# yu-changqian/TorchSeg

Hardware: AMD Instinct MI355X
Metric: training images/sec (1024x1024) BiSeNet-R18 (higher is better)
Workload: dtype bf16

## Files before the change

### torchseg_amd/csrc/conv3wrw.hip

```cpp
#include "tsg_common.h"
#include <stdlib.h>

namespace tsg {

typedef __attribute__((ext_vector_type(8))) __bf16 bf16x8;
typedef __attribute__((ext_vector_type(16))) float f32x16;
typedef uint32_t __attribute__((may_alias)) lds_u32;
typedef uint16_t __attribute__((may_alias)) lds_u16;
typedef bf16x8 __attribute__((may_alias)) lds_bf16x8;

constexpr int W3_C = 64;
constexpr int W3_N = 9 * W3_C;
constexpr int W3_TH = 4, W3_TW = 32;
constexpr int W3_PR = W3_TH + 2;
constexpr int W3_PP = (W3_TW + 2) / 2;
constexpr int W3_RD = 20;
constexpr int W3_CS = 121;
constexpr int W3_COPY = W3_C * W3_CS;
constexpr int W3_DS = 68;
constexpr int W3_NCH = 8 * W3_PR * W3_PP;
constexpr int W3_NU = (W3_NCH + 255) / 256;
constexpr int W3_NPART = 256;

struct W3Geom { int B, H, W, tiles_h, tiles_w, ntiles, two; };

__global__ __launch_bounds__(256) void conv3_wrw_k(const bf16_t* __restrict__ x, const bf16_t* __restrict__ dy,
                                                   float* __restrict__ part, W3Geom g) {
  extern __shared__ __attribute__((aligned(16))) uint32_t lds[];
  lds_u32* dyT = reinterpret_cast<lds_u32*>(lds);
  lds_u32* xT = dyT + W3_C * W3_DS;
  lds_u16* xT16 = reinterpret_cast<lds_u16*>(xT);
  const int tid = threadIdx.x, lane = tid & 63, wave = tid >> 6, half = lane >> 5, n = lane & 31;
  const int wm = wave >> 1, wh = wave & 1;

  const int spp = tid & 15, strow = (tid >> 4) & 1, spart = tid >> 5;
  int xoff[W3_NU], xrc[W3_NU], xdst[W3_NU];
#pragma unroll
  for (int u = 0; u < W3_NU; ++u) {
    const int q = tid + 256 * u;
    const int cpart = q / (W3_PR * W3_PP), rem = q % (W3_PR * W3_PP), r = rem / W3_PP, pc = rem % W3_PP;
    xrc[u] = q < W3_NCH ? (r | ((2 * pc) << 8)) : -1;
    xoff[u] = ((r - 1) * g.W + 2 * pc - 1) * W3_C + cpart * 8;
    xdst[u] = (cpart * 8) * W3_CS + r * W3_RD + pc;
  }
  const lds_u32* afrag = dyT + (32 * wm + n) * W3_DS + 4 * half;
  const lds_u32* bfrag = xT + (32 * wh + n) * W3_CS + 4 * half;

  f32x16 acc[9];
#pragma unroll
  for (int t = 0; t < 9; ++t)
#pragma unroll
    for (int r = 0; r < 16; ++r) acc[t][r] = 0.f;

  uint4 rd[4];
  uint4 rx[W3_NU][2];
  auto fetch = [&](int tile) {
    const int ow0 = (tile % g.tiles_w) * W3_TW, oh0 = ((tile / g.tiles_w) % g.tiles_h) * W3_TH;
    const int b = tile / (g.tiles_w * g.tiles_h);
    const int64_t org = (((int64_t)b * g.H + oh0) * g.W + ow0) * W3_C;
    const bf16_t* dt = dy + org + ((int64_t)strow * g.W + 2 * spp) * W3_C + spart * 8;
#pragma unroll
    for (int rs = 0; rs < 2; ++rs)
#pragma unroll
      for (int px = 0; px < 2; ++px)
        rd[rs * 2 + px] = (oh0 + strow + 2 * rs < g.H && ow0 + 2 * spp + px < g.W)
                              ? *reinterpret_cast<const uint4*>(dt + ((int64_t)rs * 2 * g.W + px) * W3_C)
                              : make_uint4(0, 0, 0, 0);
    const bf16_t* xo = x + org;
#pragma unroll
    for (int u = 0; u < W3_NU; ++u) {
      const int ih = oh0 - 1 + (xrc[u] & 0xff), iw = ow0 - 1 + (xrc[u] >> 8);
      const bool rowok = xrc[u] >= 0 && ih >= 0 && ih < g.H;
      rx[u][0] = (rowok && iw >= 0 && iw < g.W) ? *reinterpret_cast<const uint4*>(xo + xoff[u]) : make_uint4(0, 0, 0, 0);
      rx[u][1] = (rowok && iw + 1 >= 0 && iw + 1 < g.W) ? *reinterpret_cast<const uint4*>(xo + xoff[u] + W3_C)
                                                         : make_uint4(0, 0, 0, 0);
    }
  };

  int tile = blockIdx.x;
  if (tile < g.ntiles) fetch(tile);
  for (; tile < g.ntiles; tile += gridDim.x) {
    __syncthreads();
#pragma unroll
    for (int rs = 0; rs < 2; ++rs) {
      const uint32_t wa[4] = {rd[2 * rs].x, rd[2 * rs].y, rd[2 * rs].z, rd[2 * rs].w};
      const uint32_t wb[4] = {rd[2 * rs + 1].x, rd[2 * rs + 1].y, rd[2 * rs + 1].z, rd[2 * rs + 1].w};
      lds_u32* drow = dyT + (spart * 8) * W3_DS + 16 * (strow + 2 * rs) + spp;
#pragma unroll
      for (int e = 0; e < 8; ++e)
        drow[e * W3_DS] = (e & 1) ? ((wa[e >> 1] >> 16) | (wb[e >> 1] & 0xffff0000u))
                                  : ((wa[e >> 1] & 0xffffu) | (wb[e >> 1] << 16));
    }
#pragma unroll
    for (int u = 0; u < W3_NU; ++u) {
      if (u < W3_NU - 1 || xrc[u] >= 0) {
        const uint32_t wa[4] = {rx[u][0].x, rx[u][0].y, rx[u][0].z, rx[u][0].w};
        const uint32_t wb[4] = {rx[u][1].x, rx[u][1].y, rx[u][1].z, rx[u][1].w};
#pragma unroll
        for (int e = 0; e < 8; ++e) {
          const uint32_t a = (e & 1) ? (wa[e >> 1] >> 16) : (wa[e >> 1] & 0xffffu);
          const uint32_t b2 = (e & 1) ? (wb[e >> 1] >> 16) : (wb[e >> 1] & 0xffffu);
          const int d = xdst[u] + e * W3_CS;
          xT[d] = a | (b2 << 16);
          xT16[2 * (W3_COPY + d) + 1] = (uint16_t)a;
          xT16[2 * (W3_COPY + d) + g.two] = (uint16_t)b2;
        }
      }
    }
    __syncthreads();
    if (tile + (int)gridDim.x < g.ntiles) fetch(tile + gridDim.x);
#pragma unroll
    for (int ks = 0; ks < 8; ++ks) {
      const bf16x8 fa = *reinterpret_cast<const lds_bf16x8*>(afrag + ks * 8);
#pragma unroll
      for (int kh = 0; kh < 3; ++kh)
#pragma unroll
        for (int kw = 0; kw < 3; ++kw) {
          const int sg = kw & 1;
          const lds_u32* q = bfrag + sg * W3_COPY + ((ks >> 1) + kh) * W3_RD + (ks & 1) * 8 + ((kw + sg) >> 1);
          union { uint32_t u[4]; bf16x8 v; } fb;
          fb.u[0] = q[0]; fb.u[1] = q[1]; fb.u[2] = q[2]; fb.u[3] = q[3];
          acc[kh * 3 + kw] = __builtin_amdgcn_mfma_f32_32x32x16_bf16(fa, fb.v, acc[kh * 3 + kw], 0, 0, 0);
        }
    }
  }
  float* out = part + (int64_t)blockIdx.x * W3_C * W3_N;
#pragma unroll
  for (int t = 0; t < 9; ++t)
#pragma unroll
    for (int r = 0; r < 16; ++r) {
      const int oc = 32 * wm + (r & 3) + 8 * (r >> 2) + 4 * half;
      out[oc * W3_N + t * W3_C + 32 * wh + n] = acc[t][r];
    }
}

typedef short v4i16 __attribute__((ext_vector_type(4)));
typedef v4i16 __attribute__((address_space(3))) lds_v4i16;

constexpr int T3_RBE = 96;
constexpr int T3_PC = W3_TW + 2;
constexpr int T3_NPX = W3_PR * T3_PC;
constexpr int T3_DY = W3_TH * W3_TW * T3_RBE;
constexpr int T3_XU = (T3_NPX * 8 + 255) / 256;
constexpr size_t T3_LDS = (size_t)(T3_DY + T3_NPX * T3_RBE) * sizeof(bf16_t);

__device__ __forceinline__ uint4 w3_affine_relu(uint4 v, const float* __restrict__ ab, int part8) {
  uint32_t w[4] = {v.x, v.y, v.z, v.w};
  const float4 a0 = *reinterpret_cast<const float4*>(ab + part8), a1 = *reinterpret_cast<const float4*>(ab + part8 + 4);
  const float4 b0 = *reinterpret_cast<const float4*>(ab + W3_C + part8), b1 = *reinterpret_cast<const float4*>(ab + W3_C + part8 + 4);
  const float a[8] = {a0.x, a0.y, a0.z, a0.w, a1.x, a1.y, a1.z, a1.w};
  const float b[8] = {b0.x, b0.y, b0.z, b0.w, b1.x, b1.y, b1.z, b1.w};
#pragma unroll
  for (int i = 0; i < 4; ++i) {
    const float x0 = __uint_as_float(w[i] << 16), x1 = __uint_as_float(w[i] & 0xffff0000u);
    const float y0 = fmaf(x0, a[2 * i], b[2 * i]), y1 = fmaf(x1, a[2 * i + 1], b[2 * i + 1]);
    w[i] = pack2_bf16(y0 > 0.f ? y0 : 0.f, y1 > 0.f ? y1 : 0.f);
  }
  return make_uint4(w[0], w[1], w[2], w[3]);
}

template <bool AFF>
__global__ __launch_bounds__(256) void conv3_wrw_tr_k(const bf16_t* __restrict__ x, const bf16_t* __restrict__ dy,
                                                      float* __restrict__ part, W3Geom g, const float* __restrict__ in_ab) {
  __shared__ __attribute__((aligned(16))) float abs_[AFF ? 2 * W3_C : 4];
  if (AFF && threadIdx.x < 2 * W3_C) abs_[threadIdx.x] = in_ab[threadIdx.x];
  extern __shared__ __attribute__((aligned(16))) uint32_t lds[];
  bf16_t* dyL = reinterpret_cast<bf16_t*>(lds);
  bf16_t* xL = dyL + T3_DY;
  const int tid = threadIdx.x, lane = tid & 63, wave = tid >> 6;
  const int wm = wave >> 1, wh = wave & 1;
  const int half = lane >> 5, sub = (lane >> 4) & 1, i16 = lane & 15;

  const int spart = tid & 7, spix = tid >> 3;
  int xr[T3_XU], xc[T3_XU];
#pragma unroll
  for (int u = 0; u < T3_XU; ++u) {
    const int pp = spix + 32 * u;
    xr[u] = pp < T3_NPX ? pp / T3_PC : -1;
    xc[u] = pp % T3_PC;
  }
  const int fbase = (8 * half + (i16 >> 2)) * T3_RBE + 16 * sub + 4 * (i16 & 3);
  const lds_v4i16* afr = (const lds_v4i16*)(dyL + fbase + 32 * wm);
  const lds_v4i16* bfr = (const lds_v4i16*)(xL + fbase + 32 * wh);

  f32x16 acc[9];
#pragma unroll
  for (int t = 0; t < 9; ++t)
#pragma unroll
    for (int r = 0; r < 16; ++r) acc[t][r] = 0.f;

  uint4 rd[W3_TH];
  uint4 rx[T3_XU];
  auto fetch = [&](int tile) {
    const int ow0 = (tile % g.tiles_w) * W3_TW, oh0 = ((tile / g.tiles_w) % g.tiles_h) * W3_TH;
    const int b = tile / (g.tiles_w * g.tiles_h);
    const int64_t org = (((int64_t)b * g.H + oh0) * g.W + ow0) * W3_C;
    const bf16_t* dt = dy + org + (int64_t)spix * W3_C + spart * 8;
#pragma unroll
    for (int u = 0; u < W3_TH; ++u)
      rd[u] = (oh0 + u < g.H && ow0 + spix < g.W) ? *reinterpret_cast<const uint4*>(dt + (int64_t)u * g.W * W3_C)
                                                  : make_uint4(0, 0, 0, 0);
    const bf16_t* xo = x + org + spart * 8;
#pragma unroll
    for (int u = 0; u < T3_XU; ++u) {
      const int ih = oh0 - 1 + xr[u], iw = ow0 - 1 + xc[u];
      rx[u] = (xr[u] >= 0 && ih >= 0 && ih < g.H && iw >= 0 && iw < g.W)
                  ? *reinterpret_cast<const uint4*>(xo + ((int64_t)(xr[u] - 1) * g.W + xc[u] - 1) * W3_C)
                  : make_uint4(0, 0, 0, 0);
    }
  };

  int tile = blockIdx.x;
  if (tile < g.ntiles) fetch(tile);
  for (; tile < g.ntiles; tile += gridDim.x) {
    __syncthreads();
#pragma unroll
    for (int u = 0; u < W3_TH; ++u)
      *reinterpret_cast<uint4*>(dyL + (spix + 32 * u) * T3_RBE + spart * 8) = rd[u];
    const int cur_ow0 = (tile % g.tiles_w) * W3_TW, cur_oh0 = ((tile / g.tiles_w) % g.tiles_h) * W3_TH;
#pragma unroll
    for (int u = 0; u < T3_XU; ++u)
      if (u < T3_XU - 1 || xr[u] >= 0) {
        uint4 v = rx[u];
        if (AFF) {
          const int ih = cur_oh0 - 1 + xr[u], iw = cur_ow0 - 1 + xc[u];
          if (ih >= 0 && ih < g.H && iw >= 0 && iw < g.W) v = w3_affine_relu(v, abs_, spart * 8);
        }
        *reinterpret_cast<uint4*>(xL + (spix + 32 * u) * T3_RBE + spart * 8) = v;
      }
    __syncthreads();
    if (tile + (int)gridDim.x < g.ntiles) fetch(tile + gridDim.x);
#pragma unroll
    for (int ks = 0; ks < 8; ++ks) {
      union { v4i16 q[2]; bf16x8 v; } fa;
      fa.q[0] = __builtin_amdgcn_ds_read_tr16_b64_v4i16((lds_v4i16*)(afr + (ks * 16 + 0) * (T3_RBE / 4)));
      fa.q[1] = __builtin_amdgcn_ds_read_tr16_b64_v4i16((lds_v4i16*)(afr + (ks * 16 + 4) * (T3_RBE / 4)));
#pragma unroll
      for (int kh = 0; kh < 3; ++kh)
#pragma unroll
        for (int kw = 0; kw < 3; ++kw) {
          const int px = ((ks >> 1) + kh) * T3_PC + (ks & 1) * 16 + kw;
          union { v4i16 q[2]; bf16x8 v; } fb;
          fb.q[0] = __builtin_amdgcn_ds_read_tr16_b64_v4i16((lds_v4i16*)(bfr + (px + 0) * (T3_RBE / 4)));
          fb.q[1] = __builtin_amdgcn_ds_read_tr16_b64_v4i16((lds_v4i16*)(bfr + (px + 4) * (T3_RBE / 4)));
          acc[kh * 3 + kw] = __builtin_amdgcn_mfma_f32_32x32x16_bf16(fa.v, fb.v, acc[kh * 3 + kw], 0, 0, 0);
        }
    }
  }
  float* out = part + (int64_t)blockIdx.x * W3_C * W3_N;
#pragma unroll
  for (int t = 0; t < 9; ++t)
#pragma unroll
    for (int r = 0; r < 16; ++r) {
      const int oc = 32 * wm + (r & 3) + 8 * (r >> 2) + 4 * half;
      out[oc * W3_N + t * W3_C + 32 * wh + (lane & 31)] = acc[t][r];
    }
}

struct W3GenGeom {
  int B, H, W, tiles_h, tiles_w, ntiles;
  int Hin, Win;
  int Cin, Cout, nci, npairs, bpp;
  int xs;
  int prio;
};

template <int S> struct W3S {
  static constexpr int PR = S * W3_TH + 3 - S, PC = S * W3_TW + 3 - S, NPX = PR * PC;
  static constexpr int XU = (NPX * 8 + 255) / 256;
  static constexpr size_t LDS = (size_t)(T3_DY + NPX * T3_RBE) * sizeof(bf16_t);
};

template <int S, int PF, bool AFF, bool BUF = false>
__global__ __launch_bounds__(256, PF ? 1 : 2) void conv3_wrw_gen_k(const bf16_t* __restrict__ x, const bf16_t* __restrict__ dy,
                                                       float* __restrict__ part, W3GenGeom g, const float* __restrict__ in_ab) {
  typedef W3S<S> P;
  __shared__ __attribute__((aligned(16))) float abs_[AFF ? 2 * W3_C : 4];
  extern __shared__ __attribute__((aligned(16))) uint32_t lds[];
  bf16_t* dyL = reinterpret_cast<bf16_t*>(lds);
  bf16_t* xL = dyL + T3_DY;
  const int tid = threadIdx.x, lane = tid & 63, wave = tid >> 6;
  const int wm = wave >> 1, wh = wave & 1;
  const int half = lane >> 5, sub = (lane >> 4) & 1, i16 = lane & 15;
  const int xcd = blockIdx.x & 7, jb = blockIdx.x >> 3;
  const int pps = g.npairs / g.xs;
  const int pair = (g.xs == 2 ? (xcd & 1) * pps : 0) + jb % pps;
  const int slot = (jb / pps) * (8 / g.xs) + (g.xs == 2 ? xcd >> 1 : xcd);
  const int oc0 = (pair / g.nci) * W3_C, ci0 = (pair % g.nci) * W3_C;
  if (AFF && tid < 2 * W3_C) abs_[tid] = in_ab[(tid >> 6) * g.Cin + ci0 + (tid & 63)];

  const int spart = tid & 7, spix = tid >> 3;
  int xr[P::XU], xc[P::XU];
#pragma unroll
  for (int u = 0; u < P::XU; ++u) {
    const int pp = spix + 32 * u;
    xr[u] = pp < P::NPX ? pp / P::PC : -1;
    xc[u] = pp % P::PC;
  }
  const int chan = 16 * sub + 4 * (i16 & 3);
  const lds_v4i16* afr = (const lds_v4i16*)(dyL + (8 * half + (i16 >> 2)) * T3_RBE + chan + 32 * wm);
  const lds_v4i16* bfr = (const lds_v4i16*)(xL + S * (8 * half + (i16 >> 2)) * T3_RBE + chan + 32 * wh);

  f32x16 acc[9];
#pragma unroll
  for (int t = 0; t < 9; ++t)
#pragma unroll
    for (int r = 0; r < 16; ++r) acc[t][r] = 0.f;

  uint4 rd[W3_TH];
  uint4 rx[P::XU];
  uint32_t dyo[BUF ? W3_TH : 1], xo32[BUF ? P::XU : 1];
  if (BUF) {
#pragma unroll
    for (int u = 0; u < W3_TH; ++u) dyo[BUF ? u : 0] = (uint32_t)((((int64_t)u * g.W + spix) * g.Cout + spart * 8) * 2);
#pragma unroll
    for (int u = 0; u < P::XU; ++u)
      xo32[BUF ? u : 0] = (uint32_t)((((int64_t)(xr[u] < 0 ? 0 : xr[u]) * g.Win + xc[u]) * g.Cin + spart * 8) * 2);
  }
  int ftw = 0, fth = 0, fb = 0;
  const int dtw = g.bpp % g.tiles_w, dth = (g.bpp / g.tiles_w) % g.tiles_h, db = g.bpp / (g.tiles_w * g.tiles_h);
  if (BUF) { ftw = slot % g.tiles_w; fth = (slot / g.tiles_w) % g.tiles_h; fb = slot / (g.tiles_w * g.tiles_h); }
  auto fetch = [&](int tile) {
    const int ow0 = BUF ? ftw * W3_TW : (tile % g.tiles_w) * W3_TW;
    const int oh0 = BUF ? fth * W3_TH : ((tile / g.tiles_w) % g.tiles_h) * W3_TH;
    const int b = BUF ? fb : tile / (g.tiles_w * g.tiles_h);
    const int64_t pix = ((int64_t)b * g.H + oh0) * g.W + ow0;
    if (BUF) {
      constexpr uint32_t kOob = 0x80000000u;
      const int ih0 = S * oh0 - 1, iw0 = S * ow0 - 1;
      const bf16_t* dbase = dy + pix * g.Cout + oc0;
      const bf16_t* xbase = x + (((int64_t)b * g.Hin + ih0) * g.Win + iw0) * g.Cin + ci0;
      const __amdgpu_buffer_rsrc_t rd_ = __builtin_amdgcn_make_buffer_rsrc((void*)dbase, 0, 0x7fffffff, 0x00020000);
      const __amdgpu_buffer_rsrc_t rx_ = __builtin_amdgcn_make_buffer_rsrc((void*)xbase, 0, 0x7fffffff, 0x00020000);
      const bool live = tile < g.ntiles;
      const bool colok = live && ow0 + spix < g.W;
#pragma unroll
      for (int u = 0; u < W3_TH; ++u) {
        const uint32_t off = (colok && oh0 + u < g.H) ? dyo[BUF ? u : 0] : kOob;
        const u32x4 v = __builtin_amdgcn_raw_buffer_load_b128(rd_, (int)off, 0, 0);
        rd[u] = make_uint4(v.x, v.y, v.z, v.w);
      }
#pragma unroll
      for (int u = 0; u < P::XU; ++u) {
        const bool ok = live && (uint32_t)(ih0 + xr[u]) < (uint32_t)g.Hin && (uint32_t)(iw0 + xc[u]) < (uint32_t)g.Win && xr[u] >= 0;
        const uint32_t off = ok ? xo32[BUF ? u : 0] : kOob;
        const u32x4 v = __builtin_amdgcn_raw_buffer_load_b128(rx_, (int)off, 0, 0);
        rx[u] = make_uint4(v.x, v.y, v.z, v.w);
      }
      ftw += dtw; if (ftw >= g.tiles_w) { ftw -= g.tiles_w; ++fth; }
      fth += dth; if (fth >= g.tiles_h) { fth -= g.tiles_h; ++fb; }
      fb += db;
      return;
    }
    const bf16_t* dt = dy + (pix + spix) * g.Cout + oc0 + spart * 8;
#pragma unroll
    for (int u = 0; u < W3_TH; ++u)
      rd[u] = (oh0 + u < g.H && ow0 + spix < g.W) ? *reinterpret_cast<const uint4*>(dt + (int64_t)u * g.W * g.Cout)
                                                  : make_uint4(0, 0, 0, 0);
    const int ih0 = S * oh0 - 1, iw0 = S * ow0 - 1;
    const bf16_t* xo = x + (((int64_t)b * g.Hin + ih0) * g.Win + iw0) * g.Cin + ci0 + spart * 8;
#pragma unroll
    for (int u = 0; u < P::XU; ++u) {
      const int ih = ih0 + xr[u], iw = iw0 + xc[u];
      rx[u] = (xr[u] >= 0 && ih >= 0 && ih < g.Hin && iw >= 0 && iw < g.Win)
                  ? *reinterpret_cast<const uint4*>(xo + ((int64_t)xr[u] * g.Win + xc[u]) * g.Cin)
                  : make_uint4(0, 0, 0, 0);
    }
  };
  auto stage = [&](const uint4* qd_, const uint4* qx_, int tile_, bool rezero) {
    const int cur_ow0 = (tile_ % g.tiles_w) * W3_TW, cur_oh0 = ((tile_ / g.tiles_w) % g.tiles_h) * W3_TH;
#pragma unroll
    for (int u = 0; u < W3_TH; ++u) {
      uint4 v = qd_[u];
      if (rezero && !(cur_oh0 + u < g.H && cur_ow0 + spix < g.W)) v = make_uint4(0, 0, 0, 0);
      *reinterpret_cast<uint4*>(dyL + (spix + 32 * u) * T3_RBE + spart * 8) = v;
    }
#pragma unroll
    for (int u = 0; u < P::XU; ++u)
      if (u < P::XU - 1 || xr[u] >= 0) {
        uint4 v = qx_[u];
        const int ih = S * cur_oh0 - 1 + xr[u], iw = S * cur_ow0 - 1 + xc[u];
        const bool in = ih >= 0 && ih < g.Hin && iw >= 0 && iw < g.Win;
        if (AFF && in) v = w3_affine_relu(v, abs_, spart * 8);
        if (rezero && !in) v = make_uint4(0, 0, 0, 0);
        *reinterpret_cast<uint4*>(xL + (spix + 32 * u) * T3_RBE + spart * 8) = v;
      }
  };
  union Frag { v4i16 q[2]; bf16x8 v; };
  auto mfma_tile = [&]() {
    if (g.prio) __builtin_amdgcn_s_setprio(1);
    Frag fa[8];
#pragma unroll
    for (int ks = 0; ks < 8; ++ks) {
      fa[ks].q[0] = __builtin_amdgcn_ds_read_tr16_b64_v4i16((lds_v4i16*)(afr + (ks * 16 + 0) * (T3_RBE / 4)));
      fa[ks].q[1] = __builtin_amdgcn_ds_read_tr16_b64_v4i16((lds_v4i16*)(afr + (ks * 16 + 4) * (T3_RBE / 4)));
    }
#pragma unroll
    for (int pr = 0; pr < S * 3 + 3; ++pr)
#pragma unroll
      for (int c = 0; c < 2; ++c)
#pragma unroll
        for (int kw = 0; kw < 3; ++kw) {
          const int px = pr * P::PC + S * c * 16 + kw;
          Frag fb;
          fb.q[0] = __builtin_amdgcn_ds_read_tr16_b64_v4i16((lds_v4i16*)(bfr + (px + 0) * (T3_RBE / 4)));
          fb.q[1] = __builtin_amdgcn_ds_read_tr16_b64_v4i16((lds_v4i16*)(bfr + (px + 4 * S) * (T3_RBE / 4)));
#pragma unroll
          for (int kh = 0; kh < 3; ++kh) {
            const int rr = pr - kh;
            if (rr >= 0 && rr % S == 0 && rr / S < 4)
              acc[kh * 3 + kw] = __builtin_amdgcn_mfma_f32_32x32x16_bf16(fa[2 * (rr / S) + c].v, fb.v, acc[kh * 3 + kw], 0, 0, 0);
          }
        }
    if (g.prio) __builtin_amdgcn_s_setprio(0);
  };

  if (PF == 2) {
    constexpr int L = W3_TH + P::XU;
    u32x4 qd[PF == 2 ? 2 : 1][W3_TH], qx[PF == 2 ? 2 : 1][PF == 2 ? P::XU : 1];
    const int last = slot < g.ntiles ? slot + (g.ntiles - 1 - slot) / g.bpp * g.bpp : 0;
#define TSG_W3_FETCH(SET, TILE)                                                                               \
    {                                                                                                         \
      const int t_ = (TILE) < g.ntiles ? (TILE) : last;                                                       \
      const int ow0_ = (t_ % g.tiles_w) * W3_TW, oh0_ = ((t_ / g.tiles_w) % g.tiles_h) * W3_TH;               \
      const int b_ = t_ / (g.tiles_w * g.tiles_h);                                                            \
      const int64_t pix_ = ((int64_t)b_ * g.H + oh0_) * g.W + ow0_;                                           \
      const bf16_t* dt_ = dy + (pix_ + spix) * g.Cout + oc0 + spart * 8;                                      \
      _Pragma("unroll") for (int u_ = 0; u_ < W3_TH; ++u_) {                                                  \
        const bf16_t* p_ = (oh0_ + u_ < g.H && ow0_ + spix < g.W) ? dt_ + (int64_t)u_ * g.W * g.Cout : dy;    \
        TSG_ASM_LD16(qd[SET][u_], p_, 0);                                                                     \
      }                                                                                                       \
      const int ih0_ = S * oh0_ - 1, iw0_ = S * ow0_ - 1;                                                     \
      const bf16_t* xo_ = x + (((int64_t)b_ * g.Hin + ih0_) * g.Win + iw0_) * g.Cin + ci0 + spart * 8;        \
      _Pragma("unroll") for (int u_ = 0; u_ < P::XU; ++u_) {                                                  \
        const int ih_ = ih0_ + xr[u_], iw_ = iw0_ + xc[u_];                                                   \
        const bf16_t* p_ = (xr[u_] >= 0 && ih_ >= 0 && ih_ < g.Hin && iw_ >= 0 && iw_ < g.Win)                \
                               ? xo_ + ((int64_t)xr[u_] * g.Win + xc[u_]) * g.Cin : x;                        \
        TSG_ASM_LD16(qx[SET][PF == 2 ? u_ : 0], p_, 0);                                                       \
      }                                                                                                       \
    }
    int tile = slot;
    if (tile < g.ntiles) {
      TSG_W3_FETCH(0, tile)
      TSG_W3_FETCH(1, tile + g.bpp)
      for (bool more = true; more;) {
#pragma unroll
        for (int s_ = 0; s_ < 2; ++s_) {
          __syncthreads();
          vm_wait<L>(qd[PF == 2 ? s_ : 0][0]);
#pragma unroll
          for (int u = 1; u < W3_TH; ++u) vm_tie(qd[PF == 2 ? s_ : 0][u]);
#pragma unroll
          for (int u = 0; u < P::XU; ++u) vm_tie(qx[PF == 2 ? s_ : 0][PF == 2 ? u : 0]);
          uint4 td[W3_TH], tx[P::XU];
#pragma unroll
          for (int u = 0; u < W3_TH; ++u) { const u32x4 v = qd[PF == 2 ? s_ : 0][u]; td[u] = make_uint4(v.x, v.y, v.z, v.w); }
#pragma unroll
          for (int u = 0; u < P::XU; ++u) { const u32x4 v = qx[PF == 2 ? s_ : 0][PF == 2 ? u : 0]; tx[u] = make_uint4(v.x, v.y, v.z, v.w); }
          stage(td, tx, tile, true);
          __syncthreads();
          TSG_W3_FETCH(PF == 2 ? s_ : 0, tile + 2 * g.bpp)
          mfma_tile();
          tile += g.bpp;
          if (tile >= g.ntiles) { more = false; break; }
        }
      }
      asm volatile("s_waitcnt vmcnt(0)");
    }
#undef TSG_W3_FETCH
  } else {
    int tile = slot;
    if (PF == 1 && tile < g.ntiles) fetch(tile);
    for (; tile < g.ntiles; tile += g.bpp) {
      if (PF == 0) fetch(tile);
      __syncthreads();
      stage(rd, rx, tile, false);
      __syncthreads();
      if (PF == 1 && (BUF || tile + g.bpp < g.ntiles)) fetch(tile + g.bpp);
      mfma_tile();
    }
  }
  float* out = part + ((int64_t)pair * g.bpp + slot) * W3_C * W3_N;
#pragma unroll
  for (int t = 0; t < 9; ++t)
#pragma unroll
    for (int r = 0; r < 16; ++r) {
      const int oc = 32 * wm + (r & 3) + 8 * (r >> 2) + 4 * half;
      out[oc * W3_N + t * W3_C + 32 * wh + (lane & 31)] = acc[t][r];
    }
}

__global__ __launch_bounds__(256) void conv3_wrw_gen_fold(const float* __restrict__ part, W3GenGeom g,
                                                          float* __restrict__ dw) {
  __shared__ double sm[16][64];
  const int run = blockIdx.x % (W3_C * 9), pair = blockIdx.x / (W3_C * 9);
  const int oc0 = (pair / g.nci) * W3_C, ci0 = (pair % g.nci) * W3_C;
  const int c4 = threadIdx.x & 15, gs = threadIdx.x >> 4;
  const float* src = part + (int64_t)pair * g.bpp * W3_C * W3_N + run * 64 + c4 * 4;
  double a0 = 0.0, a1 = 0.0, a2 = 0.0, a3 = 0.0;
  for (int s0 = gs; s0 < g.bpp; s0 += 16 * 8) {
    float4 v[8];
#pragma unroll
    for (int u = 0; u < 8; ++u) {
      const int s = s0 + 16 * u;
      v[u] = *reinterpret_cast<const float4*>(src + (int64_t)(s < g.bpp ? s : gs) * W3_C * W3_N);
      if (s >= g.bpp) v[u] = make_float4(0.f, 0.f, 0.f, 0.f);
    }
#pragma unroll
    for (int u = 0; u < 8; ++u) { a0 += (double)v[u].x; a1 += (double)v[u].y; a2 += (double)v[u].z; a3 += (double)v[u].w; }
  }
  sm[gs][c4 * 4 + 0] = a0; sm[gs][c4 * 4 + 1] = a1; sm[gs][c4 * 4 + 2] = a2; sm[gs][c4 * 4 + 3] = a3;
  __syncthreads();
  if (threadIdx.x < 64) {
    double t = 0.0;
#pragma unroll
    for (int q = 0; q < 16; ++q) t += sm[q][threadIdx.x];
    const int oc = run / 9, tap = run % 9;
    dw[((int64_t)(oc0 + oc) * 9 + tap) * g.Cin + ci0 + threadIdx.x] = (float)t;
  }
}

__global__ __launch_bounds__(256) void conv3_wrw_gen_fold2(const float* __restrict__ part, W3GenGeom g, int T,
                                                           float* __restrict__ dw) {
  __shared__ double sm[256][4];
  const int outs = 256 / T;
  const int t = threadIdx.x / outs, o = threadIdx.x - t * outs;
  constexpr int QP = W3_C * W3_N / 4;
  const int64_t q_all = (int64_t)blockIdx.x * outs + o;
  const int pair = (int)(q_all / QP), q = (int)(q_all - (int64_t)pair * QP);
  const float* src = part + (int64_t)pair * g.bpp * W3_C * W3_N + (int64_t)q * 4;
  double a0 = 0.0, a1 = 0.0, a2 = 0.0, a3 = 0.0;
  for (int s0 = t; s0 < g.bpp; s0 += 8 * T) {
    float4 v[8];
#pragma unroll
    for (int u = 0; u < 8; ++u) {
      const int s = s0 + u * T;
      v[u] = *reinterpret_cast<const float4*>(src + (int64_t)(s < g.bpp ? s : t) * W3_C * W3_N);
      if (s >= g.bpp) v[u] = make_float4(0.f, 0.f, 0.f, 0.f);
    }
#pragma unroll
    for (int u = 0; u < 8; ++u) { a0 += (double)v[u].x; a1 += (double)v[u].y; a2 += (double)v[u].z; a3 += (double)v[u].w; }
  }
  if (T > 1) {
    sm[threadIdx.x][0] = a0; sm[threadIdx.x][1] = a1; sm[threadIdx.x][2] = a2; sm[threadIdx.x][3] = a3;
    __syncthreads();
    if (t == 0) {
      for (int k = 1; k < T; ++k) {
        const double* r = sm[k * outs + o];
        a0 += r[0]; a1 += r[1]; a2 += r[2]; a3 += r[3];
      }
    }
  }
  if (t == 0) {
    const int e = q * 4, oc = e / W3_N, rem = e - oc * W3_N, tap = rem / W3_C, ci = rem - tap * W3_C;
    const int oc0 = (pair / g.nci) * W3_C, ci0 = (pair % g.nci) * W3_C;
    *reinterpret_cast<float4*>(dw + ((int64_t)(oc0 + oc) * 9 + tap) * g.Cin + ci0 + ci) =
        make_float4((float)a0, (float)a1, (float)a2, (float)a3);
  }
}

__global__ __launch_bounds__(256) void conv3_wrw_fold(const float* __restrict__ part, int nparts, int64_t stride,
                                                      float* __restrict__ dw) {
  __shared__ double sm[16][64];
  const int c4 = threadIdx.x & 15, gs = threadIdx.x >> 4;
  const float* src = part + blockIdx.x * 64 + c4 * 4;
  double a0 = 0.0, a1 = 0.0, a2 = 0.0, a3 = 0.0;
  for (int s0 = gs; s0 < nparts; s0 += 16 * 8) {
    float4 v[8];
#pragma unroll
    for (int u = 0; u < 8; ++u) {
      const int gidx = s0 + 16 * u;
      v[u] = *reinterpret_cast<const float4*>(src + (int64_t)(gidx < nparts ? gidx : gs) * stride);
      if (gidx >= nparts) v[u] = make_float4(0.f, 0.f, 0.f, 0.f);
    }
#pragma unroll
    for (int u = 0; u < 8; ++u) { a0 += (double)v[u].x; a1 += (double)v[u].y; a2 += (double)v[u].z; a3 += (double)v[u].w; }
  }
  sm[gs][c4 * 4 + 0] = a0; sm[gs][c4 * 4 + 1] = a1; sm[gs][c4 * 4 + 2] = a2; sm[gs][c4 * 4 + 3] = a3;
  __syncthreads();
  if (threadIdx.x < 64) {
    double t = 0.0;
#pragma unroll
    for (int q = 0; q < 16; ++q) t += sm[q][threadIdx.x];
    dw[blockIdx.x * 64 + threadIdx.x] = (float)t;
  }
}

constexpr size_t W3_LDS = (size_t)(W3_C * W3_DS + 2 * W3_COPY) * sizeof(uint32_t) + 16;

}

using namespace tsg;

extern "C" {

int tsg_conv3x3_wrw_supported(int dtype, int Cin, int Cout, int kh, int kw, int stride, int pad, int dilation,
                              int groups) {
  return dtype == TSG_BF16 && Cin == W3_C && Cout == W3_C && kh == 3 && kw == 3 && stride == 1 && pad == 1 &&
         dilation == 1 && groups == 1;
}

size_t tsg_conv3x3_wrw_ws_bytes(void) { return (size_t)W3_NPART * W3_C * W3_N * sizeof(float); }

static int conv3_wrw_common(int variant, const void* x, const void* dy, float* dw, int64_t B, int64_t H, int64_t W,
                            void* ws, size_t ws_bytes, void* stream, const float* in_ab = nullptr) {
  if (!x || !dy || !dw || !ws) return TSG_E_NULL;
  if (in_ab && (variant != 1 || !aligned16(in_ab))) return in_ab && variant != 1 ? TSG_E_SHAPE : TSG_E_ALIGN;
  if (B <= 0 || H <= 0 || W <= 0) return TSG_E_SHAPE;
  const int64_t th = (H + W3_TH - 1) / W3_TH, tw = (W + W3_TW - 1) / W3_TW;
  if (B * th * tw > 0x7fffffffLL || H * W * W3_C > 0x7fffffffLL) return TSG_E_SHAPE;
  if (ws_bytes < tsg_conv3x3_wrw_ws_bytes()) return TSG_E_WS;
  if (!aligned16(x) || !aligned16(dy) || !aligned16(dw) || !aligned16(ws)) return TSG_E_ALIGN;
  W3Geom g;
  g.B = (int)B; g.H = (int)H; g.W = (int)W; g.tiles_h = (int)th; g.tiles_w = (int)tw; g.ntiles = (int)(B * th * tw); g.two = 2;
  hipStream_t st = (hipStream_t)stream;
  TSG_HIP(hipFuncSetAttribute(reinterpret_cast<const void*>(&conv3_wrw_k), hipFuncAttributeMaxDynamicSharedMemorySize,
                              (int)W3_LDS));
  const int grid = g.ntiles < W3_NPART ? g.ntiles : W3_NPART;
  if (variant == 1 && in_ab) {
    TSG_HIP(hipFuncSetAttribute(reinterpret_cast<const void*>(&conv3_wrw_tr_k<true>),
                                hipFuncAttributeMaxDynamicSharedMemorySize, (int)T3_LDS));
    hipLaunchKernelGGL(conv3_wrw_tr_k<true>, dim3(grid), dim3(256), T3_LDS, st, (const bf16_t*)x, (const bf16_t*)dy,
                       (float*)ws, g, in_ab);
  } else if (variant == 1) {
    TSG_HIP(hipFuncSetAttribute(reinterpret_cast<const void*>(&conv3_wrw_tr_k<false>),
                                hipFuncAttributeMaxDynamicSharedMemorySize, (int)T3_LDS));
    hipLaunchKernelGGL(conv3_wrw_tr_k<false>, dim3(grid), dim3(256), T3_LDS, st, (const bf16_t*)x, (const bf16_t*)dy,
                       (float*)ws, g, (const float*)nullptr);
  } else {
    hipLaunchKernelGGL(conv3_wrw_k, dim3(grid), dim3(256), W3_LDS, st, (const bf16_t*)x, (const bf16_t*)dy, (float*)ws,
                       g);
  }
  TSG_CHECK_LAUNCH();
  hipLaunchKernelGGL(conv3_wrw_fold, dim3(W3_C * W3_N / 64), dim3(256), 0, st, (const float*)ws, grid,
                     (int64_t)W3_C * W3_N, dw);
  TSG_CHECK_LAUNCH();
  return 0;
}

int tsg_conv3x3_wrw(const void* x, const void* dy, float* dw, int64_t B, int64_t H, int64_t W, void* ws,
                    size_t ws_bytes, void* stream) {
  return conv3_wrw_common(0, x, dy, dw, B, H, W, ws, ws_bytes, stream);
}

int tsg_conv3x3_wrw_tr(const void* x, const void* dy, float* dw, int64_t B, int64_t H, int64_t W, void* ws,
                       size_t ws_bytes, void* stream) {
  return conv3_wrw_common(1, x, dy, dw, B, H, W, ws, ws_bytes, stream);
}

int tsg_conv3x3_wrw_tr_norm(const void* x, const float* in_ab, const void* dy, float* dw, int64_t B, int64_t H, int64_t W,
                            void* ws, size_t ws_bytes, void* stream) {
  if (!in_ab) return TSG_E_NULL;
  return conv3_wrw_common(1, x, dy, dw, B, H, W, ws, ws_bytes, stream, in_ab);
}

static bool w3_pf2() {
  static const bool v = [] { const char* e = getenv("TSG_CONV_WRW_PF2"); return e && e[0] == '1'; }();
  return v;
}
static bool w3_occ2(int64_t ntiles) {
  static const int v = [] { const char* e = getenv("TSG_CONV_WRW_OCC"); return e ? atoi(e) : 1; }();
  return !w3_pf2() && v == 2 && ntiles >= 1024;
}

static int w3gen_geom(W3GenGeom* g, int64_t B, int64_t Hin, int64_t Win, int Cin, int Cout, int stride) {
  if (B <= 0 || Hin <= 0 || Win <= 0 || Cin <= 0 || Cout <= 0 || Cin % W3_C || Cout % W3_C) return TSG_E_SHAPE;
  if (stride != 1 && stride != 2) return TSG_E_SHAPE;
  const int64_t H = (Hin - 1) / stride + 1, W = (Win - 1) / stride + 1;
  const int64_t th = (H + W3_TH - 1) / W3_TH, tw = (W + W3_TW - 1) / W3_TW;
  if (B * th * tw > 0x7fffffffLL || B * Hin * Win * (int64_t)(Cin > Cout ? Cin : Cout) > 0x7fffffff00LL) return TSG_E_SHAPE;
  g->B = (int)B; g->H = (int)H; g->W = (int)W; g->Hin = (int)Hin; g->Win = (int)Win;
  g->tiles_h = (int)th; g->tiles_w = (int)tw; g->ntiles = (int)(B * th * tw);
  g->Cin = Cin; g->Cout = Cout; g->nci = Cin / W3_C; g->npairs = (Cout / W3_C) * g->nci;
  static int target = 0;
  if (!target) { const char* e = getenv("TSG_CONV_WRW_BLOCKS"); target = e ? atoi(e) : 256; if (target < 1) target = 256; }
  int bpp = ((stride == 1 && w3_occ2(g->ntiles) ? 2 * target : target) + g->npairs - 1) / g->npairs;
  if (bpp > g->ntiles) bpp = g->ntiles;
  if (bpp < 1) bpp = 1;
  static const bool xs2 = [] { const char* e = getenv("TSG_CONV_WRW_XS2"); return !(e && e[0] == '0'); }();
  g->xs = (xs2 && bpp <= 4 && g->npairs % 2 == 0 && g->npairs * 8 > target) ? 2 : 1;
  g->bpp = g->xs == 2 ? (bpp + 3) / 4 * 4 : (bpp + 7) / 8 * 8;
  static const int prio = [] { const char* e = getenv("TSG_MFMA_PRIO"); return e ? atoi(e) : 0; }();
  g->prio = prio;
  return 0;
}

int tsg_conv3x3_wrw_gen_supported(int dtype, int Cin, int Cout, int kh, int kw, int stride, int pad, int dilation,
                                  int groups) {
  return dtype == TSG_BF16 && Cin > 0 && Cout > 0 && Cin % W3_C == 0 && Cout % W3_C == 0 && kh == 3 && kw == 3 &&
         (stride == 1 || stride == 2) && pad == 1 && dilation == 1 && groups == 1;
}

size_t tsg_conv3x3_wrw_gen_ws_bytes(int64_t B, int64_t Hin, int64_t Win, int Cin, int Cout, int stride) {
  W3GenGeom g;
  if (w3gen_geom(&g, B, Hin, Win, Cin, Cout, stride)) return 0;
  return (size_t)g.npairs * g.bpp * W3_C * W3_N * sizeof(float);
}

static int conv3_wrw_gen_common(const void* x, const float* in_ab, const void* dy, float* dw, int64_t B, int64_t Hin,
                                int64_t Win, int Cin, int Cout, int stride, void* ws, size_t ws_bytes, void* stream) {
  if (!x || !dy || !dw || !ws) return TSG_E_NULL;
  if (in_ab && !aligned16(in_ab)) return TSG_E_ALIGN;
  W3GenGeom g;
  int e = w3gen_geom(&g, B, Hin, Win, Cin, Cout, stride);
  if (e) return e;
  if (ws_bytes < tsg_conv3x3_wrw_gen_ws_bytes(B, Hin, Win, Cin, Cout, stride)) return TSG_E_WS;
  if (!aligned16(x) || !aligned16(dy) || !aligned16(dw) || !aligned16(ws)) return TSG_E_ALIGN;
  hipStream_t st = (hipStream_t)stream;
  static const bool buf_env = [] { const char* e = getenv("TSG_CONV_WRW_BUF"); return !(e && e[0] == '0'); }();
  const bool buf = buf_env && (int64_t)(3 * stride + 4) * Win * Cin * 2 < 0x40000000LL && (int64_t)5 * g.W * Cout * 2 < 0x40000000LL;
#define W3_GO2(SS, PFF, AF, BF)                                                                                   \
  do {                                                                                                            \
    TSG_HIP(hipFuncSetAttribute(reinterpret_cast<const void*>(&conv3_wrw_gen_k<SS, PFF, AF, BF>),                 \
                                hipFuncAttributeMaxDynamicSharedMemorySize, (int)W3S<SS>::LDS));                  \
    hipLaunchKernelGGL((conv3_wrw_gen_k<SS, PFF, AF, BF>), dim3(g.npairs * g.bpp), dim3(256), W3S<SS>::LDS, st,   \
                       (const bf16_t*)x, (const bf16_t*)dy, (float*)ws, g, in_ab);                                \
  } while (0)
#define W3_GO(SS, PFF, AF) do { if (buf && PFF != 2) W3_GO2(SS, (PFF == 2 ? 1 : PFF), AF, true); else W3_GO2(SS, PFF, AF, false); } while (0)
  if (stride == 1 && w3_pf2()) { if (in_ab) W3_GO(1, 2, true); else W3_GO(1, 2, false); }
  else if (stride == 1 && w3_occ2(g.ntiles)) { if (in_ab) W3_GO(1, 0, true); else W3_GO(1, 0, false); }
  else if (stride == 1) { if (in_ab) W3_GO(1, 1, true); else W3_GO(1, 1, false); }
  else { if (in_ab) W3_GO(2, 1, true); else W3_GO(2, 1, false); }
#undef W3_GO
#undef W3_GO2
  TSG_CHECK_LAUNCH();
  static const bool fold2 = [] { const char* e = getenv("TSG_CONV_WRW_FOLD"); return !(e && e[0] == '1'); }();
  if (fold2) {
    const int T = g.bpp <= 8 ? 1 : g.bpp <= 16 ? 2 : g.bpp <= 32 ? 4 : g.bpp <= 64 ? 8 : 16;
    const int64_t blocks = (int64_t)g.npairs * (W3_C * W3_N / 4) / (256 / T);
    hipLaunchKernelGGL(conv3_wrw_gen_fold2, dim3((unsigned)blocks), dim3(256), 0, st, (const float*)ws, g, T, dw);
  } else {
    hipLaunchKernelGGL(conv3_wrw_gen_fold, dim3(g.npairs * W3_C * 9), dim3(256), 0, st, (const float*)ws, g, dw);
  }
  TSG_CHECK_LAUNCH();
  return 0;
}

int tsg_conv3x3_wrw_gen(const void* x, const void* dy, float* dw, int64_t B, int64_t Hin, int64_t Win, int Cin, int Cout,
                        int stride, void* ws, size_t ws_bytes, void* stream) {
  return conv3_wrw_gen_common(x, nullptr, dy, dw, B, Hin, Win, Cin, Cout, stride, ws, ws_bytes, stream);
}

int tsg_conv3x3_wrw_gen_norm(const void* x, const float* in_ab, const void* dy, float* dw, int64_t B, int64_t Hin,
                             int64_t Win, int Cin, int Cout, int stride, void* ws, size_t ws_bytes, void* stream) {
  if (!in_ab) return TSG_E_NULL;
  return conv3_wrw_gen_common(x, in_ab, dy, dw, B, Hin, Win, Cin, Cout, stride, ws, ws_bytes, stream);
}

}

namespace tsg {
template <typename TI>
__global__ __launch_bounds__(256) void w3_rot180_t_k(const TI* __restrict__ w, bf16_t* __restrict__ out, int O, int I) {
  __shared__ float tile[32][33];
  const int tap = blockIdx.z, o0 = blockIdx.y * 32, i0 = blockIdx.x * 32;
  const int tx = threadIdx.x & 31, ty = threadIdx.x >> 5;
  for (int r = ty; r < 32; r += 8) {
    const int o = o0 + r, i = i0 + tx;
    tile[r][tx] = (o < O && i < I) ? ld1<TI>(w + ((int64_t)o * 9 + (8 - tap)) * I + i) : 0.f;
  }
  __syncthreads();
  for (int r = ty; r < 32; r += 8) {
    const int i = i0 + r, o = o0 + tx;
    if (i < I && o < O) out[((int64_t)i * 9 + tap) * O + o] = f32_to_bf16(tile[tx][r]);
  }
}
}

extern "C" int tsg_conv3x3_weight_rot180_t(const void* w, int dtype, void* out, int O, int I, void* stream) {
  if (!w || !out) return TSG_E_NULL;
  if (O <= 0 || I <= 0) return TSG_E_SHAPE;
  if (dtype != TSG_F32 && dtype != TSG_BF16) return TSG_E_DTYPE;
  dim3 grid((unsigned)((I + 31) / 32), (unsigned)((O + 31) / 32), 9);
  if (dtype == TSG_F32)
    hipLaunchKernelGGL((tsg::w3_rot180_t_k<float>), grid, dim3(256), 0, (hipStream_t)stream, (const float*)w, (tsg::bf16_t*)out, O, I);
  else
    hipLaunchKernelGGL((tsg::w3_rot180_t_k<tsg::bf16_t>), grid, dim3(256), 0, (hipStream_t)stream, (const tsg::bf16_t*)w,
                       (tsg::bf16_t*)out, O, I);
  TSG_CHECK_LAUNCH();
  return 0;
}
```

Before: 1336.

## Add triple-buffered LDS ring pipeline for stride-1 conv3x3 weight gradient

```diff
diff --git a/torchseg_amd/csrc/conv3wrw.hip b/torchseg_amd/csrc/conv3wrw.hip
--- a/torchseg_amd/csrc/conv3wrw.hip
+++ b/torchseg_amd/csrc/conv3wrw.hip
@@ -1,5 +1,6 @@
 #include "tsg_common.h"
 #include <stdlib.h>
+#include <type_traits>
 
 namespace tsg {
 
@@ -271,9 +272,168 @@
   static constexpr size_t LDS = (size_t)(T3_DY + NPX * T3_RBE) * sizeof(bf16_t);
 };
 
+__device__ __forceinline__ void w3_pair_slot(const W3GenGeom& g, int& pair, int& slot) {
+  const int xcd = blockIdx.x & 7, jb = blockIdx.x >> 3;
+  const int pps = g.npairs / g.xs;
+  pair = (g.xs == 2 ? (xcd & 1) * pps : 0) + jb % pps;
+  slot = (jb / pps) * (8 / g.xs) + (g.xs == 2 ? xcd >> 1 : xcd);
+}
+
+constexpr int R3_DYP = W3_TH * W3_TW / 8;
+constexpr int R3_XP = 28;
+constexpr int R3_PPW = (R3_DYP + R3_XP) / 4;
+constexpr int R3_STAGE = (R3_DYP + R3_XP) * 1024;
+constexpr int R3_NST = 3;
+constexpr size_t R3_LDS = (size_t)R3_NST * R3_STAGE;
+static_assert(R3_XP * 8 >= T3_NPX && (R3_DYP + R3_XP) % 4 == 0 && R3_DYP == 16, "ring stage layout");
+
+__device__ __forceinline__ void w3_ring(const bf16_t* __restrict__ x, const bf16_t* __restrict__ dy, float* __restrict__ part,
+                                        const W3GenGeom& g) {
+  typedef unsigned char __attribute__((address_space(3))) lds_u8;
+  typedef __attribute__((address_space(3))) void* lds_ptr_t;
+  extern __shared__ __attribute__((aligned(16))) unsigned char r3_smem[];
+  lds_u8* const smem = (lds_u8*)r3_smem;
+  const int lane = threadIdx.x & 63;
+  const int wave = __builtin_amdgcn_readfirstlane(threadIdx.x >> 6);
+  const int wm = wave >> 1, wh = wave & 1;
+  const int half = lane >> 5, sub = (lane >> 4) & 1, i16 = lane & 15;
+  int pair, slot;
+  w3_pair_slot(g, pair, slot);
+  const int oc0 = (pair / g.nci) * W3_C, ci0 = (pair % g.nci) * W3_C;
+
+  const int lpart = (lane & 7) ^ (((lane >> 4) & 1) << 2);
+  const int dcol = 8 * wave + (lane >> 3);
+  uint32_t dyo[W3_TH], xo[R3_PPW - W3_TH];
+  int xrc[R3_PPW - W3_TH];
+#pragma unroll
+  for (int u = 0; u < W3_TH; ++u) dyo[u] = (uint32_t)((((int64_t)u * g.W + dcol) * g.Cout + lpart * 8) * 2);
+#pragma unroll
+  for (int v = 0; v < R3_PPW - W3_TH; ++v) {
+    const int px = 8 * (wave + 4 * v) + (lane >> 3), pr = px / T3_PC, pc = px % T3_PC;
+    xrc[v] = px < T3_NPX ? (pr | (pc << 8)) : -1;
+    xo[v] = (uint32_t)((((int64_t)pr * g.Win + pc) * g.Cin + lpart * 8) * 2);
+  }
+  const int prow = (8 * half + (i16 >> 2)) * 128 + 8 * (i16 & 1);
+  const int ch16 = 2 * sub + ((i16 >> 1) & 1);
+  const int abase = prow + ((ch16 + 4 * wm) ^ ((((i16 >> 2) >> 1) & 1) << 2)) * 16;
+  int bbase[4];
+#pragma unroll
+  for (int d = 0; d < 4; ++d) bbase[d] = R3_DYP * 1024 + prow + ((ch16 + 4 * wh) ^ (((((i16 >> 2) + d) >> 1) & 1) << 2)) * 16;
+
+  f32x16 acc[9];
+#pragma unroll
+  for (int t = 0; t < 9; ++t)
+#pragma unroll
+    for (int r = 0; r < 16; ++r) acc[t][r] = 0.f;
+
+  int ftw = slot % g.tiles_w, fth = (slot / g.tiles_w) % g.tiles_h, fb = slot / (g.tiles_w * g.tiles_h);
+  const int dtw = g.bpp % g.tiles_w, dth = (g.bpp / g.tiles_w) % g.tiles_h, db = g.bpp / (g.tiles_w * g.tiles_h);
+  const int nt = slot < g.ntiles ? (g.ntiles - 1 - slot) / g.bpp + 1 : 0;
+  __amdgpu_buffer_rsrc_t rdy, rx;
+  int ioh0 = 0, iow0 = 0;
+  bool ilive = false;
+  lds_u8* isb = smem;
+  auto prep = [&](int j, int stg) {
+    ilive = j < nt;
+    iow0 = ftw * W3_TW; ioh0 = fth * W3_TH;
+    const int64_t pix = ((int64_t)fb * g.H + ioh0) * g.W + iow0;
+    rdy = __builtin_amdgcn_make_buffer_rsrc((void*)(dy + pix * g.Cout + oc0), 0, 0x7fffffff, 0x00020000);
+    rx = __builtin_amdgcn_make_buffer_rsrc((void*)(x + (((int64_t)fb * g.Hin + ioh0 - 1) * g.Win + iow0 - 1) * g.Cin + ci0), 0,
+                                           0x7fffffff, 0x00020000);
+    isb = smem + stg * R3_STAGE;
+    ftw += dtw; if (ftw >= g.tiles_w) { ftw -= g.tiles_w; ++fth; }
+    fth += dth; if (fth >= g.tiles_h) { fth -= g.tiles_h; ++fb; }
+    fb += db;
+  };
+  auto piece = [&](int u) {
+    constexpr uint32_t kOob = 0x80000000u;
+    if (u < W3_TH) {
+      const uint32_t off = (ilive && iow0 + dcol < g.W && ioh0 + u < g.H) ? dyo[u < W3_TH ? u : 0] : kOob;
+      __builtin_amdgcn_raw_ptr_buffer_load_lds(rdy, (lds_ptr_t)(isb + (wave + 4 * u) * 1024), 16, (int)off, 0, 0, 0);
+    } else {
+      const int v = u < W3_TH ? 0 : u - W3_TH;
+      const bool ok = ilive && xrc[v] >= 0 && (uint32_t)(ioh0 - 1 + (xrc[v] & 0xff)) < (uint32_t)g.Hin &&
+                      (uint32_t)(iow0 - 1 + (xrc[v] >> 8)) < (uint32_t)g.Win;
+      __builtin_amdgcn_raw_ptr_buffer_load_lds(rx, (lds_ptr_t)(isb + (R3_DYP + wave + 4 * v) * 1024), 16,
+                                               (int)(ok ? xo[v] : kOob), 0, 0, 0);
+    }
+  };
+  union Frag { v4i16 q[2]; bf16x8 v; };
+  auto mfma_tile = [&](const lds_u8* sb) {
+    if (g.prio) __builtin_amdgcn_s_setprio(1);
+    Frag fa[8];
+#pragma unroll
+    for (int ks = 0; ks < 8; ++ks) {
+      fa[ks].q[0] = __builtin_amdgcn_ds_read_tr16_b64_v4i16((lds_v4i16*)(sb + abase + (ks * 16 + 0) * 128));
+      fa[ks].q[1] = __builtin_amdgcn_ds_read_tr16_b64_v4i16((lds_v4i16*)(sb + abase + (ks * 16 + 4) * 128));
+    }
+    Frag fb_[2][3];
+    auto read_step = [&](int j, Frag* f) {
+      const int pr = j >> 1, c = j & 1;
+#pragma unroll
+      for (int kw = 0; kw < 3; ++kw) {
+        const int px = pr * T3_PC + c * 16 + kw;
+        const lds_u8* bq = sb + bbase[(2 * pr + kw) & 3];
+        f[kw].q[0] = __builtin_amdgcn_ds_read_tr16_b64_v4i16((lds_v4i16*)(bq + (px + 0) * 128));
+        f[kw].q[1] = __builtin_amdgcn_ds_read_tr16_b64_v4i16((lds_v4i16*)(bq + (px + 4) * 128));
+      }
+    };
+    read_step(0, fb_[0]);
+#pragma unroll
+    for (int j = 0; j < 12; ++j) {
+      const int pr = j >> 1, c = j & 1;
+      if (j + 1 < 12) read_step(j + 1, fb_[(j + 1) & 1]);
+      if (j < R3_PPW) piece(j);
+      __builtin_amdgcn_sched_barrier(0);
+#pragma unroll
+      for (int kw = 0; kw < 3; ++kw)
+#pragma unroll
+        for (int kh = 0; kh < 3; ++kh) {
+          const int rr = pr - kh;
+          if (rr >= 0 && rr < 4)
+            acc[kh * 3 + kw] = __builtin_amdgcn_mfma_f32_32x32x16_bf16(fa[2 * rr + c].v, fb_[j & 1][kw].v, acc[kh * 3 + kw], 0, 0, 0);
+        }
+      __builtin_amdgcn_sched_barrier(0);
+    }
+    if (g.prio) __builtin_amdgcn_s_setprio(0);
+  };
+
+  if (nt > 0) {
+    prep(0, 0);
+#pragma unroll
+    for (int u = 0; u < R3_PPW; ++u) piece(u);
+    prep(1, 1);
+#pragma unroll
+    for (int u = 0; u < R3_PPW; ++u) piece(u);
+  }
+  int st = 0;
+  for (int i = 0; i < nt; ++i) {
+    static_assert(R3_PPW == 11, "the counted wait");
+    asm volatile("s_waitcnt vmcnt(11) lgkmcnt(0)\n\ts_barrier" ::: "memory");
+    prep(i + 2, st == 0 ? 2 : st - 1);
+    lds_u8* sb = smem + st * R3_STAGE;
+    mfma_tile(sb);
+    st = st == 2 ? 0 : st + 1;
+  }
+  asm volatile("s_waitcnt vmcnt(0)" ::: "memory");
+  float* out = part + ((int64_t)pair * g.bpp + slot) * W3_C * W3_N;
+#pragma unroll
+  for (int t = 0; t < 9; ++t)
+#pragma unroll
+    for (int r = 0; r < 16; ++r) {
+      const int oc = 32 * wm + (r & 3) + 8 * (r >> 2) + 4 * half;
+      out[oc * W3_N + t * W3_C + 32 * wh + (lane & 31)] = acc[t][r];
+    }
+}
+
 template <int S, int PF, bool AFF, bool BUF = false>
 __global__ __launch_bounds__(256, PF ? 1 : 2) void conv3_wrw_gen_k(const bf16_t* __restrict__ x, const bf16_t* __restrict__ dy,
                                                        float* __restrict__ part, W3GenGeom g, const float* __restrict__ in_ab) {
+  if constexpr (PF == 3) {
+    static_assert(S == 1 && !AFF, "the ring stages plain stride-1 tiles");
+    w3_ring(x, dy, part, g);
+    return;
+  }
   typedef W3S<S> P;
   __shared__ __attribute__((aligned(16))) float abs_[AFF ? 2 * W3_C : 4];
   extern __shared__ __attribute__((aligned(16))) uint32_t lds[];
@@ -282,10 +442,8 @@
   const int tid = threadIdx.x, lane = tid & 63, wave = tid >> 6;
   const int wm = wave >> 1, wh = wave & 1;
   const int half = lane >> 5, sub = (lane >> 4) & 1, i16 = lane & 15;
-  const int xcd = blockIdx.x & 7, jb = blockIdx.x >> 3;
-  const int pps = g.npairs / g.xs;
-  const int pair = (g.xs == 2 ? (xcd & 1) * pps : 0) + jb % pps;
-  const int slot = (jb / pps) * (8 / g.xs) + (g.xs == 2 ? xcd >> 1 : xcd);
+  int pair, slot;
+  w3_pair_slot(g, pair, slot);
   const int oc0 = (pair / g.nci) * W3_C, ci0 = (pair % g.nci) * W3_C;
   if (AFF && tid < 2 * W3_C) abs_[tid] = in_ab[(tid >> 6) * g.Cin + ci0 + (tid & 63)];
 
@@ -662,6 +820,10 @@
   static const int v = [] { const char* e = getenv("TSG_CONV_WRW_OCC"); return e ? atoi(e) : 1; }();
   return !w3_pf2() && v == 2 && ntiles >= 1024;
 }
+static bool w3_ring() {
+  static const bool v = [] { const char* e = getenv("TSG_CONV_WRW_RING"); return !(e && e[0] == '0'); }();
+  return v;
+}
 
 static int w3gen_geom(W3GenGeom* g, int64_t B, int64_t Hin, int64_t Win, int Cin, int Cout, int stride) {
   if (B <= 0 || Hin <= 0 || Win <= 0 || Cin <= 0 || Cout <= 0 || Cin % W3_C || Cout % W3_C) return TSG_E_SHAPE;
@@ -708,7 +870,9 @@
   if (!aligned16(x) || !aligned16(dy) || !aligned16(dw) || !aligned16(ws)) return TSG_E_ALIGN;
   hipStream_t st = (hipStream_t)stream;
   static const bool buf_env = [] { const char* e = getenv("TSG_CONV_WRW_BUF"); return !(e && e[0] == '0'); }();
-  const bool buf = buf_env && (int64_t)(3 * stride + 4) * Win * Cin * 2 < 0x40000000LL && (int64_t)5 * g.W * Cout * 2 < 0x40000000LL;
+  const bool fits = (int64_t)(3 * stride + 4) * Win * Cin * 2 < 0x40000000LL && (int64_t)5 * g.W * Cout * 2 < 0x40000000LL;
+  const bool buf = buf_env && fits;
+  const bool ring = stride == 1 && fits && w3_ring();
 #define W3_GO2(SS, PFF, AF, BF)                                                                                   \
   do {                                                                                                            \
     TSG_HIP(hipFuncSetAttribute(reinterpret_cast<const void*>(&conv3_wrw_gen_k<SS, PFF, AF, BF>),                 \
@@ -717,12 +881,21 @@
                        (const bf16_t*)x, (const bf16_t*)dy, (float*)ws, g, in_ab);                                \
   } while (0)
 #define W3_GO(SS, PFF, AF) do { if (buf && PFF != 2) W3_GO2(SS, (PFF == 2 ? 1 : PFF), AF, true); else W3_GO2(SS, PFF, AF, false); } while (0)
+#define W3_RING(AF)                                                                                               \
+  do {                                                                                                            \
+    TSG_HIP(hipFuncSetAttribute(reinterpret_cast<const void*>(&conv3_wrw_gen_k<1, 3, AF, true>),                  \
+                                hipFuncAttributeMaxDynamicSharedMemorySize, (int)R3_LDS));                        \
+    hipLaunchKernelGGL((conv3_wrw_gen_k<1, 3, AF, true>), dim3(g.npairs * g.bpp), dim3(256), R3_LDS, st,          \
+                       (const bf16_t*)x, (const bf16_t*)dy, (float*)ws, g, in_ab);                                \
+  } while (0)
   if (stride == 1 && w3_pf2()) { if (in_ab) W3_GO(1, 2, true); else W3_GO(1, 2, false); }
   else if (stride == 1 && w3_occ2(g.ntiles)) { if (in_ab) W3_GO(1, 0, true); else W3_GO(1, 0, false); }
+  else if (ring && !in_ab) W3_RING(false);
   else if (stride == 1) { if (in_ab) W3_GO(1, 1, true); else W3_GO(1, 1, false); }
   else { if (in_ab) W3_GO(2, 1, true); else W3_GO(2, 1, false); }
 #undef W3_GO
 #undef W3_GO2
+#undef W3_RING
   TSG_CHECK_LAUNCH();
   static const bool fold2 = [] { const char* e = getenv("TSG_CONV_WRW_FOLD"); return !(e && e[0] == '1'); }();
   if (fold2) {
```

Result: no change. 1348 (median of 6 runs) (+0.8%).
